# akuhara/RF_INV

Measured on NVIDIA B200. Metric: forward+likelihood evals/sec, higher is better.
Workload: dtype f64

## Files before the change

### rf_inv_b200/csrc/capi.cu

```cuda
#include <cstdarg>
#include <cstdio>
#include <cstdlib>
#include <cstring>
#include <cmath>
#include <vector>
#include <algorithm>
#include "rfinv_handle.h"

static thread_local char g_err[1024] = "";

int rfinv_pdl_mode() {
  static const int mode = getenv("RFINV_PDL") ? atoi(getenv("RFINV_PDL")) : 2;
  return mode;
}

int rfinv_arith_switches() {
  auto on = [](const char* name) { return getenv(name) && atoi(getenv(name)) != 0; };
  static const int bits = (on("RFINV_FULL_BAND") ? 1 : 0) | (on("RFINV_QF_DENSE") ? 2 : 0) | (on("RFINV_QF_NOSPLIT") ? 4 : 0);
  return bits;
}

void rfinv_set_error(const char* fmt, ...) {
  va_list ap;
  va_start(ap, fmt);
// ... 365 lines not shown
  h->h_ipha.assign(cfg->ipha, cfg->ipha + T);
  h->h_obs.assign(cfg->obs, cfg->obs + (size_t)T * S);
  h->h_vp_ref.assign(cfg->vp_ref, cfg->vp_ref + cfg->nref);
  h->h_vs_ref.assign(cfg->vs_ref, cfg->vs_ref + cfg->nref);
  h->h_sig_min.assign(cfg->sig_min, cfg->sig_min + T);
  h->h_sig_max.assign(cfg->sig_max, cfg->sig_max + T);
  if (cfg->r_inv) h->h_r_inv.assign(cfg->r_inv, cfg->r_inv + (size_t)T * S * S);
  else build_r_inv(*cfg, h->h_r_inv);
  h->cfg.rayps = h->h_rayps.data(); h->cfg.a_gus = h->h_a_gus.data(); h->cfg.ipha = h->h_ipha.data();
  h->cfg.obs = h->h_obs.data(); h->cfg.vp_ref = h->h_vp_ref.data(); h->cfg.vs_ref = h->h_vs_ref.data();
  h->cfg.sig_min = h->h_sig_min.data(); h->cfg.sig_max = h->h_sig_max.data(); h->cfg.r_inv = h->h_r_inv.data();

  DevConfig& d = h->dc;
  std::memset(&d, 0, sizeof(d));
  d.ntrc = T; d.nfft = cfg->nfft; d.nh = cfg->nfft / 2 + 1; d.nsmp = S;
  d.nfft_p2 = 64; while (d.nfft_p2 < cfg->nfft) d.nfft_p2 <<= 1;
  d.fft_general = d.nfft_p2 != cfg->nfft;
  d.fft_len = d.fft_general ? 2 * d.nfft_p2 : cfg->nfft;
  d.log2n = 0; while ((1 << d.log2n) < d.fft_len) ++d.log2n;
  d.deconv_mode = cfg->deconv_mode; d.vp_mode = cfg->vp_mode; d.k_min = cfg->k_min; d.k_max = cfg->k_max;
  d.prior_mode = cfg->prior_mode; d.nref = cfg->nref;
  d.ray_common = 1;
  for (int t = 1; t < T; ++t)
    if (cfg->rayps[t] != cfg->rayps[0] || cfg->ipha[t] != cfg->ipha[0]) d.ray_common = 0;
  d.nsmp_pad = ((S + 63) / 64) * 64;
  d.delta = cfg->delta; d.t_start = cfg->t_start; d.sdep = cfg->sdep; d.bdep = cfg->bdep; d.z_ref_min = cfg->z_ref_min; d.dz_ref = cfg->dz_ref;
  d.z_min = cfg->z_min; d.z_max = cfg->z_max; d.h_min = cfg->h_min;
  d.vp_min = cfg->vp_min; d.vp_max = cfg->vp_max; d.vs_min = cfg->vs_min; d.vs_max = cfg->vs_max;
  d.vpvs_min = cfg->vpvs_min; d.vpvs_max = cfg->vpvs_max;
  d.domg = 2.0 * RFINV_PI / (cfg->nfft * cfg->delta);
  for (int t = 0; t < T; ++t) { d.rayp[t] = cfg->rayps[t]; d.ipha[t] = cfg->ipha[t]; }

  std::vector<double> flt;
  build_filter(*cfg, flt);
  band_limits(d, flt);
  std::vector<double2> tw;
  build_twiddles(d.fft_len, tw);
  std::vector<double2> chirp, chirp_b;
  std::vector<double2> twq;
  if (d.fft_general) {
    build_chirp(cfg->nfft, d.fft_len, chirp, chirp_b);
    for (int N = d.fft_len; N > 8; N >>= 3) {
      const int stride = N >> 3, tmul = d.fft_len / N;
      for (int i = 0; i < 7 * stride; ++i) { const int q = i / stride + 1, o = i - (q - 1) * stride; twq.push_back(tw[(size_t)q * o * tmul]); }
    }
  }
  const int Sp = d.nsmp_pad;
  std::vector<double> rpad((size_t)T * Sp * Sp, 0.0);
  for (int t = 0; t < T; ++t)
    for (int i = 0; i < S; ++i)
      for (int j = 0; j < S; ++j)
        rpad[((size_t)t * Sp + i) * Sp + j] =
            0.5 * (h->h_r_inv[((size_t)t * S + i) * S + j] + h->h_r_inv[((size_t)t * S + j) * S + i]);
  std::vector<double> wfac;
  {
    const bool force_dense = (rfinv_arith_switches() & 2) != 0;
    const bool no_split = (rfinv_arith_switches() & 4) != 0;
    const int ntile_dense = Sp / 64;
    std::vector<std::vector<double>> Wt(T);
    std::vector<int> wrows_t(T, 0);
    std::vector<double> a, w, v, a2, w2, v2;
    d.qf_tiles_max = 0;
    int wrows = 64;
    const double rs2 = 0.70710678118654752440;
    for (int t = 0; t < T; ++t) {
      d.qf_rank[t] = 0; d.qf_rank_s[t] = 0; d.qf_split[t] = 0;
      d.qf_tiles[t] = ntile_dense;
      const double* Rm = &rpad[(size_t)t * Sp * Sp];
      auto R = [&](int i, int j) { return Rm[(size_t)i * Sp + j]; };
      int same = -1;
      for (int u = 0; u < t && same < 0; ++u)
        if (std::memcmp(&rpad[(size_t)u * Sp * Sp], Rm, sizeof(double) * (size_t)Sp * Sp) == 0) same = u;
      if (force_dense) {  }
      else if (same >= 0) {
        d.qf_rank[t] = d.qf_rank[same]; d.qf_rank_s[t] = d.qf_rank_s[same]; d.qf_split[t] = d.qf_split[same];
        d.qf_tiles[t] = d.qf_tiles[same]; Wt[t] = Wt[same]; wrows_t[t] = wrows_t[same];
      } else {
        double rmax = 0.0, asym = 0.0;
        for (int i = 0; i < S; ++i)
          for (int j = 0; j < S; ++j) {
            rmax = std::max(rmax, std::fabs(R(i, j)));
            asym = std::max(asym, std::fabs(R(i, j) - R(S - 1 - i, S - 1 - j)));
          }
        const int ha = S / 2, hs = S - ha;
        const bool split = !no_split && rmax > 0.0 && asym <= 1e-10 * rmax && hs <= Sp / 2;
        const double units_dense = 0.5 * ntile_dense * (ntile_dense + 1);
        auto tile_units = [&](int r) { return r / 64 + (r % 64 ? 0.4 : 0.0); };
        if (split) {
          a.assign((size_t)hs * hs, 0.0); a2.assign((size_t)ha * ha, 0.0);
          for (int i = 0; i < ha; ++i)
            for (int j = 0; j < ha; ++j) {
              const int ir = S - 1 - i, jr = S - 1 - j;
              a[(size_t)i * hs + j] = 0.5 * ((R(i, j) + R(ir, jr)) + (R(i, jr) + R(ir, j)));
              a2[(size_t)i * ha + j] = 0.5 * ((R(i, j) + R(ir, jr)) - (R(i, jr) + R(ir, j)));
            }
          if (hs > ha) {
            const int c = ha;
            a[(size_t)c * hs + c] = R(c, c);
            for (int i = 0; i < ha; ++i) a[(size_t)i * hs + c] = a[(size_t)c * hs + i] = rs2 * (R(i, c) + R(S - 1 - i, c));
          }
          sym_eigh(a, hs, w, v);
          if (ha > 0) sym_eigh(a2, ha, w2, v2); else { w2.clear(); v2.clear(); }
          double lmax = 0.0, lmin = 0.0;
          for (double x : w) { lmax = std::max(lmax, x); lmin = std::min(lmin, x); }
          for (double x : w2) { lmax = std::max(lmax, x); lmin = std::min(lmin, x); }
          const double tol = 1e-12 * lmax;
          std::vector<int> os, oa;
// ... 7 lines not shown
            d.qf_rank[t] = rs + ra; d.qf_rank_s[t] = rs; d.qf_split[t] = 1;
            d.qf_tiles[t] = ts + ta;
            wrows_t[t] = 64 * (ts + ta);
            Wt[t].assign((size_t)wrows_t[t] * Sp, 0.0);
            for (int row = 0; row < rs; ++row) {
              const int e = os[row];
              const double sc = std::sqrt(w[e]);
              double* dst = &Wt[t][(size_t)row * Sp];
              for (int i = 0; i < ha; ++i) dst[i] = sc * rs2 * v[(size_t)i * hs + e];
              if (hs > ha) dst[ha] = sc * v[(size_t)ha * hs + e];
            }
            for (int row = 0; row < ra; ++row) {
              const int e = oa[row];
              const double sc = std::sqrt(w2[e]);
              double* dst = &Wt[t][(size_t)(64 * ts + row) * Sp + Sp / 2];
              for (int i = 0; i < ha; ++i) dst[i] = sc * rs2 * v2[(size_t)i * ha + e];
            }
          }
        }
        if (d.qf_rank[t] == 0 && rmax > 0.0) {
          a.resize((size_t)S * S);
          for (int i = 0; i < S; ++i)
            for (int j = 0; j < S; ++j) a[(size_t)i * S + j] = R(i, j);
          sym_eigh(a, S, w, v);
          double lmax = 0.0, lmin = 0.0;
          for (int e = 0; e < S; ++e) { lmax = std::max(lmax, w[e]); lmin = std::min(lmin, w[e]); }
          const double tol = 1e-12 * lmax;
          int r = 0;
          for (int e = 0; e < S; ++e) r += w[e] > tol;
          if (lmax > 0.0 && lmin >= -tol && r > 0 && tile_units(r) * ntile_dense < 0.9 * units_dense) {
            d.qf_rank[t] = r;
            d.qf_tiles[t] = (r + 63) / 64;
            wrows_t[t] = 64 * d.qf_tiles[t];
            Wt[t].assign((size_t)wrows_t[t] * Sp, 0.0);
            std::vector<int> order;
            for (int e = 0; e < S; ++e) if (w[e] > tol) order.push_back(e);
            std::sort(order.begin(), order.end(), [&](int x, int y) { return w[x] > w[y] || (w[x] == w[y] && x < y); });
            for (int row = 0; row < r; ++row) {
              const int e = order[row];
              const double sc = std::sqrt(w[e]);
              for (int i = 0; i < S; ++i) Wt[t][(size_t)row * Sp + i] = sc * v[(size_t)i * S + e];
            }
          }
        }
      }
      d.qf_tiles_max = std::max(d.qf_tiles_max, d.qf_tiles[t]);
      wrows = std::max(wrows, wrows_t[t]);
    }
    d.qf_wrows = wrows;
    wfac.assign((size_t)T * wrows * Sp, 0.0);
    for (int t = 0; t < T; ++t)
      if (!Wt[t].empty()) std::memcpy(&wfac[(size_t)t * wrows * Sp], Wt[t].data(), sizeof(double) * Wt[t].size());
    {
      int tr = 0;
      for (int t = 0; t < T; ++t) if (d.qf_tiles[t] > d.qf_tiles[tr]) tr = t;
      std::vector<std::pair<double, int>> cost;
      for (int jt = 0; jt < d.qf_tiles_max && jt < RFINV_MAX_QF_TILES; ++jt) {
        double cst;
        if (d.qf_rank[tr] == 0) cst = jt + 1;
        else if (d.qf_split[tr]) {
          const int rs = d.qf_rank_s[tr], ts = (rs + 63) / 64;
          cst = std::min(64, jt < ts ? rs - 64 * jt : (d.qf_rank[tr] - rs) - 64 * (jt - ts));
        } else cst = std::min(64, d.qf_rank[tr] - 64 * jt);
        cost.push_back({-cst, jt});
      }
      std::sort(cost.begin(), cost.end());
      for (size_t q = 0; q < cost.size(); ++q) d.qf_order[q] = cost[q].second;
    }
  }
#define RFINV_TRY(x) do { st = (x); if (st != RFINV_OK) { rfinv_destroy(h); return st; } } while (0)
  RFINV_TRY(upload(flt, &h->d_flt));
  RFINV_TRY(upload(tw, &h->d_tw));
  if (d.fft_general) { RFINV_TRY(upload(chirp, &h->d_chirp)); RFINV_TRY(upload(chirp_b, &h->d_chirp_b)); RFINV_TRY(upload(twq, &h->d_twq)); }
  RFINV_TRY(upload(h->h_obs, &h->d_obs));
  RFINV_TRY(upload(h->h_vp_ref, &h->d_vp_ref));
  RFINV_TRY(upload(h->h_vs_ref, &h->d_vs_ref));
  RFINV_TRY(upload(rpad, &h->d_r_inv));
  RFINV_TRY(upload(wfac, &h->d_w_fac));
#undef RFINV_TRY
  d.flt = h->d_flt; d.tw = h->d_tw; d.chirp = h->d_chirp; d.chirp_b = h->d_chirp_b; d.twq = h->d_twq; d.obs = h->d_obs; d.vp_ref = h->d_vp_ref; d.vs_ref = h->d_vs_ref; d.r_inv = h->d_r_inv; d.w_fac = h->d_w_fac;
  cudaError_t e = cudaStreamCreateWithFlags(&h->stream, cudaStreamNonBlocking);
  if (e != cudaSuccess) { rfinv_set_error("cudaStreamCreate: %s", cudaGetErrorString(e)); rfinv_destroy(h); return RFINV_ERR_CUDA; }
  h->own_stream = true;
  *out = h;
  return RFINV_OK;
}

void rfinv_destroy(rfinv_handle* h) {
  if (!h) return;
  cudaSetDevice(h->device);
  if (h->stream) cudaStreamSynchronize(h->stream);
  h->free_pt();
  rfinv_comm_destroy(h);
  h->free_workspace();
  cudaFree(h->d_flt); cudaFree(h->d_tw); cudaFree(h->d_chirp); cudaFree(h->d_chirp_b); cudaFree(h->d_twq); cudaFree(h->d_obs); cudaFree(h->d_vp_ref); cudaFree(h->d_vs_ref); cudaFree(h->d_r_inv); cudaFree(h->d_w_fac);
  if (h->own_stream && h->stream) cudaStreamDestroy(h->stream);
  if (h->stream_copy) {
    cudaStreamSynchronize(h->stream_copy);
    cudaStreamDestroy(h->stream_copy);
    for (cudaEvent_t e : h->ev_copy) if (e) cudaEventDestroy(e);
  }
  for (int i = 0; i < RFINV_ASYNC_SLOTS; ++i) {
    if (h->async_stream[i]) { cudaStreamSynchronize(h->async_stream[i]); cudaStreamDestroy(h->async_stream[i]); }
    if (h->async_ws[i]) { h->async_ws[i]->release(); delete h->async_ws[i]; }
  }
  for (int i = 0; i < 4; ++i)
    if (h->ev[i]) cudaEventDestroy(h->ev[i]);
  delete h;
}

int32_t rfinv_set_stream(rfinv_handle* h, uint64_t cuda_stream) {
  if (!h) { rfinv_set_error("handle is NULL"); return RFINV_ERR_ARG; }
  if (h->own_stream && h->stream) { cudaStreamSynchronize(h->stream); cudaStreamDestroy(h->stream); }
  h->stream = reinterpret_cast<cudaStream_t>(cuda_stream);
  h->own_stream = false;
  return RFINV_OK;
}

int32_t rfinv_synchronize(rfinv_handle* h) {
  if (!h) { rfinv_set_error("handle is NULL"); return RFINV_ERR_ARG; }
  RFINV_CUDA_CHECK(cudaStreamSynchronize(h->stream));
  return RFINV_OK;
}

int32_t rfinv_last_launch_count(rfinv_handle* h) { return h ? h->launches : 0; }

int32_t rfinv_set_timing(rfinv_handle* h, int32_t enable) {
  if (!h) { rfinv_set_error("handle is NULL"); return RFINV_ERR_ARG; }
  RFINV_CUDA_CHECK(cudaSetDevice(h->device));
  if (enable && !h->ev[0])
    for (int i = 0; i < 4; ++i) RFINV_CUDA_CHECK(cudaEventCreate(&h->ev[i]));
  h->timing = enable != 0;
  return RFINV_OK;
}

int32_t rfinv_get_quadform_form(rfinv_handle* h, int32_t* rank, int32_t* rank_s, int32_t* split) {
  if (!h || !rank || !rank_s || !split) { rfinv_set_error("rfinv_get_quadform_form: NULL argument"); return RFINV_ERR_ARG; }
  for (int t = 0; t < h->dc.ntrc; ++t) { rank[t] = h->dc.qf_rank[t]; rank_s[t] = h->dc.qf_rank_s[t]; split[t] = h->dc.qf_split[t]; }
  return RFINV_OK;
}

int32_t rfinv_get_timing(rfinv_handle* h, double* ms) {
  if (!h || !ms) { rfinv_set_error("NULL argument"); return RFINV_ERR_ARG; }
  if (!h->timing) { rfinv_set_error("rfinv_get_timing: call rfinv_set_timing(h, 1) first"); return RFINV_ERR_STATE; }
  RFINV_CUDA_CHECK(cudaEventSynchronize(h->ev[3]));
  for (int i = 0; i < 3; ++i) {
    float f = 0.f;
    RFINV_CUDA_CHECK(cudaEventElapsedTime(&f, h->ev[i], h->ev[i + 1]));
// ... 305 lines not shown
```

### rf_inv_b200/csrc/likelihood.cu

```cuda
#include "rfinv_common.cuh"

namespace {

constexpr int TM = 64;
constexpr int TN = 64;
constexpr int TK = 16;
constexpr int LDS_STRIDE = TK + 4;
constexpr int QF_THREADS = 128;
constexpr int QF_CHUNK = 384;

__device__ __forceinline__ void cp_async16(void* smem_dst, const void* gmem_src) {
  const unsigned d = (unsigned)__cvta_generic_to_shared(smem_dst);
  asm volatile("cp.async.cg.shared.global [%0], [%1], 16;\n" ::"r"(d), "l"(gmem_src));
}
__device__ __forceinline__ void cp_async_commit() { asm volatile("cp.async.commit_group;\n" ::); }
template <int N>
__device__ __forceinline__ void cp_async_wait() { asm volatile("cp.async.wait_group %0;\n" ::"n"(N)); }

__device__ __forceinline__ void dmma884(double& c0, double& c1, double a, double b) {
  asm volatile("mma.sync.aligned.m8n8k4.row.col.f64.f64.f64.f64 {%0,%1}, {%2}, {%3}, {%0,%1};\n"
               : "+d"(c0), "+d"(c1) : "d"(a), "d"(b));
}

__global__ void __launch_bounds__(QF_THREADS, 4) quadform_kernel(const DevConfig cfg, int C, const double* __restrict__ misfit,
                                                              double* __restrict__ phi, double* __restrict__ partial,
                                                              int* __restrict__ arrivals, int* __restrict__ work,
                                                              const int* __restrict__ active, int n_active,
                                                              const int* __restrict__ n_active_dev, const double* __restrict__ sig,
                                                              double* __restrict__ logl) {
  __shared__ __align__(16) double sA[2][TM * LDS_STRIDE];
  __shared__ __align__(16) double sB[2][TN * LDS_STRIDE];
  __shared__ int s_rows[TM];
  __shared__ double s_part[2][TM];
  __shared__ int s_next, s_last;
  const int Sp = cfg.nsmp_pad, T = cfg.ntrc;
  const int tid = threadIdx.x, lane = tid & 31, warp = tid >> 5;
  const int wm = warp >> 1, wn = warp & 1;
  const int n_rb_grid = ((active ? n_active : C) + TM - 1) / TM;
  const int ntile = cfg.qf_tiles_max;
  const int n_items = ntile * T * n_rb_grid;
  const int fr = lane >> 2, fk = lane & 3;
  if (tid == 0) s_next = (int)gridDim.x + atomicAdd(work, 1);
  pdl_wait();
  const int n_rows = active ? (n_active_dev ? *n_active_dev : n_active) : C;
  int item = blockIdx.x;
  while (item < n_items) {
    const int nblk = T * n_rb_grid;
    const int chunk = item / (ntile * QF_CHUNK), local = item - chunk * (ntile * QF_CHUNK);
    const int cb = min(QF_CHUNK, nblk - chunk * QF_CHUNK);
    const int jt = cfg.qf_order[local / cb];
    const int blk = chunk * QF_CHUNK + local % cb;
    const int t = blk / n_rb_grid, rb = blk - t * n_rb_grid;
    const int row0 = rb * TM;
    const int rank = cfg.qf_rank[t];
    const int ntile_t = cfg.qf_tiles[t];
    __syncthreads();
    const int next = s_next;
    int next_raw = 0;
    if (tid == 0) next_raw = atomicAdd(work, 1);
    if (row0 < n_rows && jt < ntile_t) {
      if (tid < TM) {
        int r = row0 + tid;
        r = r < n_rows ? r : n_rows - 1;
        s_rows[tid] = active ? active[r] : r;
      }
      __syncthreads();
      const double* __restrict__ Mt = misfit + (size_t)t * C * Sp;
      const double* __restrict__ Rt = rank > 0 ? cfg.w_fac + (size_t)t * cfg.qf_wrows * Sp : cfg.r_inv + (size_t)t * Sp * Sp;
      int jw = 4, koff = 0, nk = (jt + 1) * (TN / TK);
      if (rank > 0) {
        int cols_tile = rank - jt * TN;
        nk = Sp / TK;
        if (cfg.qf_split[t]) {
          const int rs = cfg.qf_rank_s[t], ts = (rs + TN - 1) / TN;
          cols_tile = jt < ts ? rs - jt * TN : (rank - rs) - (jt - ts) * TN;
          koff = jt < ts ? 0 : Sp >> 1;
          nk = (Sp >> 1) / TK;
        }
        const int nfrag = cols_tile >= TN ? 8 : (cols_tile <= 0 ? 0 : (cols_tile + 7) >> 3);
        jw = (nfrag + 1 - wn) >> 1;
      }
      const double* a_src[4];
      int cp_off[4], cp_row[4];
#pragma unroll
      for (int q = 0; q < 4; ++q) {
        const int id = tid + q * QF_THREADS;
        const int row = id >> 3, seg = id & 7;
        cp_row[q] = row;
        cp_off[q] = row * LDS_STRIDE + seg * 2;
        a_src[q] = Mt + (size_t)s_rows[row] * Sp + seg * 2 + koff;
      }
      double acc[4][4][2];
#pragma unroll
      for (int i = 0; i < 4; ++i)
#pragma unroll
        for (int j = 0; j < 4; ++j) acc[i][j][0] = acc[i][j][1] = 0.0;
      const double* b_base = Rt + (size_t)(jt * TN) * Sp + koff;
#pragma unroll
      for (int q = 0; q < 4; ++q) {
        cp_async16(&sA[0][cp_off[q]], a_src[q]);
        cp_async16(&sB[0][cp_off[q]], b_base + (size_t)cp_row[q] * Sp + (cp_off[q] - cp_row[q] * LDS_STRIDE));
      }
      cp_async_commit();
      for (int ks = 0; ks < nk; ++ks) {
        const int cur = ks & 1;
        cp_async_wait<0>();
        __syncthreads();
        if (ks + 1 < nk) {
          const int k0 = (ks + 1) * TK;
#pragma unroll
          for (int q = 0; q < 4; ++q) {
            cp_async16(&sA[cur ^ 1][cp_off[q]], a_src[q] + k0);
            cp_async16(&sB[cur ^ 1][cp_off[q]], b_base + (size_t)cp_row[q] * Sp + k0 + (cp_off[q] - cp_row[q] * LDS_STRIDE));
          }
          cp_async_commit();
        }
        if (rank == 0 && ks == jt * (TN / TK) && jt > 0) {
#pragma unroll
          for (int i = 0; i < 4; ++i)
#pragma unroll
            for (int j = 0; j < 4; ++j) { acc[i][j][0] *= 2.0; acc[i][j][1] *= 2.0; }
        }
        const double* A = &sA[cur][(wm * 32 + fr) * LDS_STRIDE + fk];
        const double* B = &sB[cur][(wn * 8 + fr) * LDS_STRIDE + fk];
#pragma unroll
        for (int kk = 0; kk < TK; kk += 4) {
          double a[4], b[4];
#pragma unroll
          for (int i = 0; i < 4; ++i) a[i] = A[i * 8 * LDS_STRIDE + kk];
#pragma unroll
          for (int j = 0; j < 4; ++j) b[j] = B[j * 16 * LDS_STRIDE + kk];
          if (jw == 4) {
#pragma unroll
            for (int i = 0; i < 4; ++i)
#pragma unroll
              for (int j = 0; j < 4; ++j) dmma884(acc[i][j][0], acc[i][j][1], a[i], b[j]);
          } else {
#pragma unroll
            for (int j = 0; j < 4; ++j)
              if (j < jw) {
#pragma unroll
                for (int i = 0; i < 4; ++i) dmma884(acc[i][j][0], acc[i][j][1], a[i], b[j]);
              }
          }
        }
      }
#pragma unroll
      for (int i = 0; i < 4; ++i) {
        const double* mrow = Mt + (size_t)s_rows[wm * 32 + 8 * i + fr] * Sp + jt * TN + wn * 8 + 2 * fk;
        double v = 0.0;
        if (rank > 0) {
#pragma unroll
          for (int j = 0; j < 4; ++j) { v = fma(acc[i][j][0], acc[i][j][0], v); v = fma(acc[i][j][1], acc[i][j][1], v); }
        } else {
#pragma unroll
          for (int j = 0; j < 4; ++j) {
            const double2 m = *reinterpret_cast<const double2*>(mrow + 16 * j);
            v = fma(acc[i][j][0], m.x, v);
            v = fma(acc[i][j][1], m.y, v);
          }
        }
        v += __shfl_xor_sync(0xffffffffu, v, 1);
        v += __shfl_xor_sync(0xffffffffu, v, 2);
        if (fk == 0) s_part[wn][wm * 32 + 8 * i + fr] = v;
      }
      __syncthreads();
      double* part_t = partial + (size_t)t * C;
      const size_t jstride = (size_t)T * C;
      if (tid < TM && row0 + tid < n_rows) part_t[(size_t)jt * jstride + s_rows[tid]] = s_part[0][tid] + s_part[1][tid];
      __threadfence();
      __syncthreads();
      if (tid == 0) s_last = (atomicAdd(&arrivals[t * n_rb_grid + rb], 1) == ntile_t - 1);
      __syncthreads();
      if (s_last) {
        __threadfence();
        if (tid < TM && row0 + tid < n_rows) {
          const int c = s_rows[tid];
          double v = 0.0;
          for (int j = 0; j < ntile_t; ++j) v += __ldcg(part_t + (size_t)j * jstride + c);
          phi[(size_t)t * C + c] = v;
        }
        if (tid == 0) arrivals[t * n_rb_grid + rb] = 0;
        if (logl) {
          __threadfence();
          __syncthreads();
          if (tid == 0) s_last = (atomicAdd(&arrivals[T * n_rb_grid + rb], 1) == T - 1);
          __syncthreads();
          if (s_last) {
            __threadfence();
            if (tid < TM && row0 + tid < n_rows) {
              const int c = s_rows[tid];
              double ll = 0.0;
              for (int tt = 0; tt < T; ++tt) {
                const double sg = sig[(size_t)tt * C + c];
                const double ph = __ldcg(phi + (size_t)tt * C + c);
                ll = __dsub_rn(__dsub_rn(ll, __ddiv_rn(__dmul_rn(0.5, ph), __dmul_rn(sg, sg))), __dmul_rn((double)cfg.nsmp, log(sg)));
              }
              logl[c] = ll;
            }
            if (tid == 0) arrivals[T * n_rb_grid + rb] = 0;
          }
        }
      }
    } else {
      __syncthreads();
    }
    if (tid == 0) s_next = (int)gridDim.x + next_raw;
    item = next;
  }
  if (tid == 0) {
    __threadfence();
    if (atomicAdd(work + 1, 1) == (int)gridDim.x - 1) { work[0] = 0; work[1] = 0; }
  }
}

__global__ void loglik_kernel(const DevConfig cfg, int C, const double* __restrict__ phi, const double* __restrict__ sig,
                              double* __restrict__ logl) {
  const int c = blockIdx.x * blockDim.x + threadIdx.x;
  if (c >= C) return;
  double ll = 0.0;
  for (int t = 0; t < cfg.ntrc; ++t) {
    const double s = sig[(size_t)t * C + c];
    const double ph = phi[(size_t)t * C + c];
    ll = __dsub_rn(__dsub_rn(ll, __ddiv_rn(__dmul_rn(0.5, ph), __dmul_rn(s, s))), __dmul_rn((double)cfg.nsmp, log(s)));
  }
  logl[c] = ll;
}

}

size_t rfinv_quadform_partial_doubles(const DevConfig& cfg, int C) { return (size_t)(cfg.nsmp_pad / TN + 1) * cfg.ntrc * C; }
size_t rfinv_quadform_counter_ints(const DevConfig& cfg, int C) { return (size_t)((C + TM - 1) / TM) * (cfg.ntrc + 1) + 4; }

int rfinv_launch_quadform(const DevConfig& cfg, int C, const double* misfit, double* phi, double* partial, int* counters,
                          const int* active, int n_active, const int* n_active_dev, cudaStream_t stream, const double* sig,
                          double* logl) {
  const int n_rows = active ? n_active : C;
  if (n_rows == 0) return RFINV_OK;
  const size_t ntile = cfg.qf_tiles_max;
  int* work = counters;
  int* arrivals = counters + 4;
  static int resident_of_device[64] = {0};
  int dev = 0;
  RFINV_CUDA_CHECK(cudaGetDevice(&dev));
  long long resident = (dev >= 0 && dev < 64) ? resident_of_device[dev] : 0;
  if (resident == 0) {
    int per_sm = 0, n_sm = 0;
    RFINV_CUDA_CHECK(cudaDeviceGetAttribute(&n_sm, cudaDevAttrMultiProcessorCount, dev));
    RFINV_CUDA_CHECK(cudaOccupancyMaxActiveBlocksPerMultiprocessor(&per_sm, quadform_kernel, QF_THREADS, 0));
    resident = (long long)n_sm * (per_sm < 1 ? 1 : per_sm);
    if (dev >= 0 && dev < 64) resident_of_device[dev] = (int)resident;
  }
  const long long items = (long long)ntile * cfg.ntrc * ((n_rows + TM - 1) / TM);
  RFINV_CUDA_CHECK(rfinv_launch_pdl(2, quadform_kernel, dim3((unsigned)(items < resident ? items : resident)), dim3(QF_THREADS), 0, stream, cfg, C,
                                    misfit, phi, partial, arrivals, work, active, n_active, n_active_dev, sig, logl));
  return RFINV_OK;
}

int rfinv_launch_loglik(const DevConfig& cfg, int C, const double* phi, const double* sig, double* logl,
                        cudaStream_t stream) {
  if (C == 0) return RFINV_OK;
  loglik_kernel<<<(C + 255) / 256, 256, 0, stream>>>(cfg, C, phi, sig, logl);
  RFINV_CUDA_CHECK(cudaGetLastError());
  return RFINV_OK;
}
```

### rf_inv_b200/csrc/rfinv_common.cuh

```cuda
#pragma once
#include <cuda_runtime.h>
#include <stdint.h>
#include <math.h>
#include <map>
#include <mutex>
#include <utility>
#include "../../include/rfinv_b200.h"

#define RFINV_MAX_TRC 16
#define RFINV_MAX_K 64
#define RFINV_MAX_LAY (RFINV_MAX_K + 2)
#define RFINV_MAX_QF_TILES 64

#define RFINV_PI 3.1415926535897931

struct DevConfig {
  int ntrc, nfft, nh, nsmp;
  int log2n;
  int fft_general, nfft_p2, fft_len;
  int deconv_mode, vp_mode, k_min, k_max, prior_mode, nref, ray_common;
  int nsmp_pad;
  double bdep;
  double delta, t_start, sdep, z_ref_min, dz_ref, z_min, z_max, h_min;
  double vp_min, vp_max, vs_min, vs_max, vpvs_min, vpvs_max;
  double domg;
  double rayp[RFINV_MAX_TRC];
  int ipha[RFINV_MAX_TRC];
  int jbins[RFINV_MAX_TRC];
  int jb_max;
  const double* flt;
  const double2* tw;
  const double2* twq;
  const double2* chirp;
  const double2* chirp_b;
  const double* obs;
  const double* vp_ref;
  const double* vs_ref;
  const double* r_inv;
  const double* w_fac;
  int qf_rank[RFINV_MAX_TRC];
  int qf_split[RFINV_MAX_TRC];
  int qf_rank_s[RFINV_MAX_TRC];
  int qf_tiles[RFINV_MAX_TRC];
  int qf_tiles_max, qf_wrows;
  int qf_order[RFINV_MAX_QF_TILES];
};

struct ModelBatch {
  int C;
  const int* k;
  const double* z;
  const double* dvp;
  const double* dvs;
  const double* sig;
  const int* active;
  int n_active;
  const int* n_active_dev;
  int chain_major = 0;
};

__host__ __device__ __forceinline__ int f_nint(double x) {
  return x >= 0.0 ? (int)floor(x + 0.5) : -(int)floor(-x + 0.5);
}

__device__ __forceinline__ double vp_to_rho(double a1) {
  double a2 = __dmul_rn(a1, a1), a3 = __dmul_rn(a2, a1), a4 = __dmul_rn(a3, a1), a5 = __dmul_rn(a4, a1);
  double p = __dmul_rn((double)1.6612f, a1);
  p = __dsub_rn(p, __dmul_rn((double)0.4721f, a2));
  p = __dadd_rn(p, __dmul_rn((double)0.0671f, a3));
  p = __dsub_rn(p, __dmul_rn((double)0.0043f, a4));
  p = __dadd_rn(p, __dmul_rn((double)0.000106f, a5));
  return p;
}

__device__ __forceinline__ bool layer_velocity(const DevConfig& cfg, double zc, double d_vs, double d_vp, double& alpha,
                                               double& beta) {
  int iz = f_nint(__ddiv_rn(__dsub_rn(zc, cfg.z_ref_min), cfg.dz_ref)) + 1;
  iz = iz < 1 ? 1 : (iz > cfg.nref ? cfg.nref : iz);
  beta = __dadd_rn(cfg.vs_ref[iz - 1], d_vs);
  alpha = cfg.vp_mode == 1 ? __dadd_rn(cfg.vp_ref[iz - 1], d_vp) : cfg.vp_ref[iz - 1];
  double ratio = __ddiv_rn(alpha, beta);
  return !(alpha < cfg.vp_min || alpha > cfg.vp_max || beta < cfg.vs_min || beta > cfg.vs_max ||
           ratio < cfg.vpvs_min || ratio > cfg.vpvs_max);
}

#define RFINV_CUDA_CHECK(expr)                                                        \
  do {                                                                                \
    cudaError_t e__ = (expr);                                                         \
    if (e__ != cudaSuccess) {                                                         \
      rfinv_set_error("%s:%d: %s -> %s", __FILE__, __LINE__, #expr, cudaGetErrorString(e__)); \
      return RFINV_ERR_CUDA;                                                          \
    }                                                                                 \
  } while (0)

void rfinv_set_error(const char* fmt, ...);

inline cudaError_t rfinv_raise_smem_limit(const void* kernel, size_t bytes) {
  static std::mutex mu;
// ... 55 lines not shown
```

### rf_inv_b200/csrc/rfinv_handle.h

```cpp
#pragma once
#include <vector>
#include "rfinv_common.cuh"

struct PtState;

struct EvalWorkspace {
  int cap = 0;
  int* d_k = nullptr;
  double *d_z = nullptr, *d_dvp = nullptr, *d_dvs = nullptr, *d_sig = nullptr, *d_stage = nullptr;
  double *d_misfit = nullptr, *d_phi = nullptr, *d_logl = nullptr, *d_rft_full = nullptr, *d_scratch = nullptr;
  uint8_t* d_valid = nullptr;
  double* d_qpart = nullptr;
  int* d_qcnt = nullptr;
  size_t cap_rft_full = 0;
  int grow(const DevConfig& dc, const rfinv_config& cfg, int device, int C);
  void release();
};

constexpr int RFINV_ASYNC_SLOTS = 2;
constexpr int RFINV_UPLOAD_PIECES = 4;

struct rfinv_handle : EvalWorkspace {
  int device = 0;
  cudaStream_t stream = nullptr;
  bool own_stream = false;
  rfinv_config cfg;
  std::vector<double> h_rayps, h_a_gus, h_obs, h_vp_ref, h_vs_ref, h_sig_min, h_sig_max, h_r_inv;
  std::vector<int32_t> h_ipha;
  DevConfig dc;
  double* d_flt = nullptr;
  double2* d_tw = nullptr;
  double2 *d_chirp = nullptr, *d_chirp_b = nullptr, *d_twq = nullptr;
  double* d_obs = nullptr;
  double* d_vp_ref = nullptr;
  double* d_vs_ref = nullptr;
  double* d_r_inv = nullptr;
  double* d_w_fac = nullptr;
  cudaStream_t stream_copy = nullptr;
  cudaEvent_t ev_copy[RFINV_UPLOAD_PIECES + 2] = {};
  EvalWorkspace* async_ws[RFINV_ASYNC_SLOTS] = {};
  cudaStream_t async_stream[RFINV_ASYNC_SLOTS] = {};
  bool async_pending[RFINV_ASYNC_SLOTS] = {};
  int launches = 0;
  bool timing = false;
  cudaEvent_t ev[4] = {nullptr, nullptr, nullptr, nullptr};
  PtState* pt = nullptr;
  void* comm = nullptr;
  int comm_world = 1, comm_rank = 0;

  int ensure_capacity(int C) { if (C > cap) invalidate_pt_graphs(); return grow(dc, cfg, device, C); }
  void invalidate_pt_graphs();
  void free_workspace() { release(); }
  void free_pt();
  int eval_device(int C, const int* k, const double* z, const double* dvp, const double* dvs, const double* sig,
                  double* logl, double* rft_smp, double* rft_full, uint8_t* is_valid, const int* active, int n_active,
                  const ModelBatch* layout = nullptr, EvalWorkspace* w = nullptr, cudaStream_t s = nullptr,
                  bool prep_done = false,
                  cudaEvent_t before_quadform = nullptr);
};

int rfinv_comm_allgather(rfinv_handle* h, const double* send, double* recv, size_t count, cudaStream_t s);
extern "C" int32_t rfinv_comm_destroy(rfinv_handle* h);
int rfinv_comm_peer_setup(rfinv_handle* h);
void rfinv_comm_peer_release(rfinv_handle* h);
int rfinv_pt_fix_assigned_bins(rfinv_handle* h);
int rfinv_pt_reserve_lhist(rfinv_handle* h, int upto);
int rfinv_arith_switches();
```

Baseline: 12.93 million.

## Emulate FP64 low-rank quadratic form with int8 tcgen05 slice GEMMs

Adds a new quadform kernel for low-rank factored traces. The misfit rows and precomputed weight factors are split into 7 int8 byte slices with per-row and per-column exponent scaling, multiplied on Blackwell tcgen05 int8 MMA into TMEM, and recombined into doubles. Rows holding non-finite values fall back to an exact FP64 loop. The old DMMA kernel now handles only dense traces, and the two kernels split the fused logl reduction. This aims to replace slow FP64 tensor-core throughput with much faster int8 throughput. It costs preprocessing, extra launch complexity and possible accuracy differences from truncating the fixed-point slices.

```diff
diff --git a/rf_inv_b200/csrc/capi.cu b/rf_inv_b200/csrc/capi.cu
--- a/rf_inv_b200/csrc/capi.cu
+++ b/rf_inv_b200/csrc/capi.cu
@@ -441,7 +441,8 @@
       for (int j = 0; j < S; ++j)
         rpad[((size_t)t * Sp + i) * Sp + j] =
             0.5 * (h->h_r_inv[((size_t)t * S + i) * S + j] + h->h_r_inv[((size_t)t * S + j) * S + i]);
-  std::vector<double> wfac;
+  std::vector<double> wfac, wcolf;
+  std::vector<uint8_t> wi8;
   {
     const bool force_dense = (rfinv_arith_switches() & 2) != 0;
     const bool no_split = (rfinv_arith_switches() & 4) != 0;
@@ -555,6 +556,31 @@
     for (int t = 0; t < T; ++t)
       if (!Wt[t].empty()) std::memcpy(&wfac[(size_t)t * wrows * Sp], Wt[t].data(), sizeof(double) * Wt[t].size());
     {
+      const int ntw = wrows / 64, nks = Sp / 32;
+      wi8.assign((size_t)T * ntw * nks * 7 * 2048, 0);
+      wcolf.assign((size_t)T * wrows, 0.0);
+      for (int t = 0; t < T; ++t) {
+        if (d.qf_rank[t] == 0) continue;
+        for (int e = 0; e < wrows; ++e) {
+          const double* col = &wfac[((size_t)t * wrows + e) * Sp];
+          double mx = 0.0;
+          for (int k = 0; k < Sp; ++k) mx = std::max(mx, std::fabs(col[k]));
+          if (mx == 0.0) continue;
+          int ec = 0;
+          std::frexp(mx, &ec);
+          wcolf[(size_t)t * wrows + e] = std::ldexp(1.0, ec - 30);
+          const int jt = e / 64, c = e % 64;
+          for (int k = 0; k < Sp; ++k) {
+            const long long X = std::llrint(std::ldexp(col[k], 55 - ec));
+            const int ks = k / 32, kb = k % 32;
+            uint8_t* blk = &wi8[(((size_t)t * ntw + jt) * nks + ks) * 7 * 2048];
+            const size_t off = (size_t)(c / 8) * 256 + (kb / 16) * 128 + (c % 8) * 16 + kb % 16;
+            for (int p = 0; p < 7; ++p) blk[(size_t)p * 2048 + off] = (uint8_t)((unsigned long long)X >> (8 * (6 - p)));
+          }
+        }
+      }
+    }
+    {
       int tr = 0;
       for (int t = 0; t < T; ++t) if (d.qf_tiles[t] > d.qf_tiles[tr]) tr = t;
       std::vector<std::pair<double, int>> cost;
@@ -580,8 +606,11 @@
   RFINV_TRY(upload(h->h_vs_ref, &h->d_vs_ref));
   RFINV_TRY(upload(rpad, &h->d_r_inv));
   RFINV_TRY(upload(wfac, &h->d_w_fac));
+  RFINV_TRY(upload(wi8, &h->d_w_i8));
+  RFINV_TRY(upload(wcolf, &h->d_w_colf));
 #undef RFINV_TRY
   d.flt = h->d_flt; d.tw = h->d_tw; d.chirp = h->d_chirp; d.chirp_b = h->d_chirp_b; d.twq = h->d_twq; d.obs = h->d_obs; d.vp_ref = h->d_vp_ref; d.vs_ref = h->d_vs_ref; d.r_inv = h->d_r_inv; d.w_fac = h->d_w_fac;
+  d.w_i8 = h->d_w_i8; d.w_colf = h->d_w_colf;
   cudaError_t e = cudaStreamCreateWithFlags(&h->stream, cudaStreamNonBlocking);
   if (e != cudaSuccess) { rfinv_set_error("cudaStreamCreate: %s", cudaGetErrorString(e)); rfinv_destroy(h); return RFINV_ERR_CUDA; }
   h->own_stream = true;
@@ -597,6 +626,7 @@
   rfinv_comm_destroy(h);
   h->free_workspace();
   cudaFree(h->d_flt); cudaFree(h->d_tw); cudaFree(h->d_chirp); cudaFree(h->d_chirp_b); cudaFree(h->d_twq); cudaFree(h->d_obs); cudaFree(h->d_vp_ref); cudaFree(h->d_vs_ref); cudaFree(h->d_r_inv); cudaFree(h->d_w_fac);
+  cudaFree(h->d_w_i8); cudaFree(h->d_w_colf);
   if (h->own_stream && h->stream) cudaStreamDestroy(h->stream);
   if (h->stream_copy) {
     cudaStreamSynchronize(h->stream_copy);
diff --git a/rf_inv_b200/csrc/likelihood.cu b/rf_inv_b200/csrc/likelihood.cu
--- a/rf_inv_b200/csrc/likelihood.cu
+++ b/rf_inv_b200/csrc/likelihood.cu
@@ -58,7 +58,7 @@
     const int next = s_next;
     int next_raw = 0;
     if (tid == 0) next_raw = atomicAdd(work, 1);
-    if (row0 < n_rows && jt < ntile_t) {
+    if (row0 < n_rows && jt < ntile_t && rank == 0) {
       if (tid < TM) {
         int r = row0 + tid;
         r = r < n_rows ? r : n_rows - 1;
@@ -66,20 +66,8 @@
       }
       __syncthreads();
       const double* __restrict__ Mt = misfit + (size_t)t * C * Sp;
-      const double* __restrict__ Rt = rank > 0 ? cfg.w_fac + (size_t)t * cfg.qf_wrows * Sp : cfg.r_inv + (size_t)t * Sp * Sp;
-      int jw = 4, koff = 0, nk = (jt + 1) * (TN / TK);
-      if (rank > 0) {
-        int cols_tile = rank - jt * TN;
-        nk = Sp / TK;
-        if (cfg.qf_split[t]) {
-          const int rs = cfg.qf_rank_s[t], ts = (rs + TN - 1) / TN;
-          cols_tile = jt < ts ? rs - jt * TN : (rank - rs) - (jt - ts) * TN;
-          koff = jt < ts ? 0 : Sp >> 1;
-          nk = (Sp >> 1) / TK;
-        }
-        const int nfrag = cols_tile >= TN ? 8 : (cols_tile <= 0 ? 0 : (cols_tile + 7) >> 3);
-        jw = (nfrag + 1 - wn) >> 1;
-      }
+      const double* __restrict__ Rt = cfg.r_inv + (size_t)t * Sp * Sp;
+      const int nk = (jt + 1) * (TN / TK);
       const double* a_src[4];
       int cp_off[4], cp_row[4];
 #pragma unroll
@@ -88,14 +76,14 @@
         const int row = id >> 3, seg = id & 7;
         cp_row[q] = row;
         cp_off[q] = row * LDS_STRIDE + seg * 2;
-        a_src[q] = Mt + (size_t)s_rows[row] * Sp + seg * 2 + koff;
+        a_src[q] = Mt + (size_t)s_rows[row] * Sp + seg * 2;
       }
       double acc[4][4][2];
 #pragma unroll
       for (int i = 0; i < 4; ++i)
 #pragma unroll
         for (int j = 0; j < 4; ++j) acc[i][j][0] = acc[i][j][1] = 0.0;
-      const double* b_base = Rt + (size_t)(jt * TN) * Sp + koff;
+      const double* b_base = Rt + (size_t)(jt * TN) * Sp;
 #pragma unroll
       for (int q = 0; q < 4; ++q) {
         cp_async16(&sA[0][cp_off[q]], a_src[q]);
@@ -115,7 +103,7 @@
           }
           cp_async_commit();
         }
-        if (rank == 0 && ks == jt * (TN / TK) && jt > 0) {
+        if (ks == jt * (TN / TK) && jt > 0) {
 #pragma unroll
           for (int i = 0; i < 4; ++i)
 #pragma unroll
@@ -130,35 +118,21 @@
           for (int i = 0; i < 4; ++i) a[i] = A[i * 8 * LDS_STRIDE + kk];
 #pragma unroll
           for (int j = 0; j < 4; ++j) b[j] = B[j * 16 * LDS_STRIDE + kk];
-          if (jw == 4) {
-#pragma unroll
-            for (int i = 0; i < 4; ++i)
-#pragma unroll
-              for (int j = 0; j < 4; ++j) dmma884(acc[i][j][0], acc[i][j][1], a[i], b[j]);
-          } else {
-#pragma unroll
-            for (int j = 0; j < 4; ++j)
-              if (j < jw) {
-#pragma unroll
-                for (int i = 0; i < 4; ++i) dmma884(acc[i][j][0], acc[i][j][1], a[i], b[j]);
-              }
-          }
+#pragma unroll
+          for (int i = 0; i < 4; ++i)
+#pragma unroll
+            for (int j = 0; j < 4; ++j) dmma884(acc[i][j][0], acc[i][j][1], a[i], b[j]);
         }
       }
 #pragma unroll
       for (int i = 0; i < 4; ++i) {
         const double* mrow = Mt + (size_t)s_rows[wm * 32 + 8 * i + fr] * Sp + jt * TN + wn * 8 + 2 * fk;
         double v = 0.0;
-        if (rank > 0) {
-#pragma unroll
-          for (int j = 0; j < 4; ++j) { v = fma(acc[i][j][0], acc[i][j][0], v); v = fma(acc[i][j][1], acc[i][j][1], v); }
-        } else {
-#pragma unroll
-          for (int j = 0; j < 4; ++j) {
-            const double2 m = *reinterpret_cast<const double2*>(mrow + 16 * j);
-            v = fma(acc[i][j][0], m.x, v);
-            v = fma(acc[i][j][1], m.y, v);
-          }
+#pragma unroll
+        for (int j = 0; j < 4; ++j) {
+          const double2 m = *reinterpret_cast<const double2*>(mrow + 16 * j);
+          v = fma(acc[i][j][0], m.x, v);
+          v = fma(acc[i][j][1], m.y, v);
         }
         v += __shfl_xor_sync(0xffffffffu, v, 1);
         v += __shfl_xor_sync(0xffffffffu, v, 2);
@@ -227,33 +201,373 @@
   logl[c] = ll;
 }
 
+
+constexpr int Q8_TM = 128;
+constexpr int Q8_TN = 64;
+constexpr int Q8_TK = 32;
+constexpr int Q8_SL = 7;
+constexpr int Q8_THREADS = 256;
+constexpr int Q8_STAGES = 3;
+constexpr int Q8_CHUNK = 192;
+constexpr int Q8_A_BYTES = Q8_TM * Q8_TK;
+constexpr int Q8_B_BYTES = Q8_TN * Q8_TK;
+constexpr int Q8_STAGE_BYTES = Q8_SL * (Q8_A_BYTES + Q8_B_BYTES);
+constexpr int Q8_SMEM = Q8_STAGES * Q8_STAGE_BYTES;
+constexpr uint32_t Q8_TMEM_COLS = 512;
+#ifndef RFINV_Q8_LBO
+#define RFINV_Q8_LBO 128
+#endif
+#ifndef RFINV_Q8_SBO
+#define RFINV_Q8_SBO 256
+#endif
+constexpr uint32_t Q8_IDESC = (2u << 4) | ((uint32_t)(Q8_TN >> 3) << 17) | ((uint32_t)(Q8_TM >> 4) << 24);
+
+__device__ __forceinline__ uint32_t smem_u32(const void* p) { return (uint32_t)__cvta_generic_to_shared(p); }
+__device__ __forceinline__ uint64_t umma_desc(uint32_t saddr) {
+  return (uint64_t)((saddr & 0x3FFFFu) >> 4) | ((uint64_t)(RFINV_Q8_LBO >> 4) << 16) | ((uint64_t)(RFINV_Q8_SBO >> 4) << 32) |
+         (1ull << 46);
+}
+__device__ __forceinline__ void mbar_wait(uint64_t* bar, uint32_t parity) {
+  const uint32_t a = smem_u32(bar);
+  uint32_t done = 0;
+  do {
+    asm volatile("{\n.reg .pred p;\nmbarrier.try_wait.parity.shared::cta.b64 p, [%1], %2;\nselp.u32 %0, 1, 0, p;\n}\n"
+                 : "=r"(done) : "r"(a), "r"(parity) : "memory");
+  } while (!done);
+}
+__device__ __forceinline__ void tc_fence_before() { asm volatile("tcgen05.fence::before_thread_sync;" ::: "memory"); }
+__device__ __forceinline__ void tc_fence_after() { asm volatile("tcgen05.fence::after_thread_sync;" ::: "memory"); }
+__device__ __forceinline__ void mma_i8(uint32_t d_tmem, uint64_t a_desc, uint64_t b_desc, uint32_t idesc, uint32_t acc) {
+  asm volatile("{\n.reg .pred p;\nsetp.ne.b32 p, %4, 0;\ntcgen05.mma.cta_group::1.kind::i8 [%0], %1, %2, %3, p;\n}\n"
+               :: "r"(d_tmem), "l"(a_desc), "l"(b_desc), "r"(idesc), "r"(acc) : "memory");
+}
+__device__ __forceinline__ void tmem_ld8(uint32_t taddr, int (&v)[8]) {
+  asm volatile("tcgen05.ld.sync.aligned.32x32b.x8.b32 {%0, %1, %2, %3, %4, %5, %6, %7}, [%8];"
+               : "=r"(v[0]), "=r"(v[1]), "=r"(v[2]), "=r"(v[3]), "=r"(v[4]), "=r"(v[5]), "=r"(v[6]), "=r"(v[7]) : "r"(taddr));
+}
+__device__ __forceinline__ double i2d_exact(long long x) {
+  return __longlong_as_double(0x4338000000000000LL + x) - 6755399441055744.0;
+}
+
+__global__ void __launch_bounds__(Q8_THREADS, 1) quadform_i8_kernel(const DevConfig cfg, int C, const double* __restrict__ misfit,
+                                                                 double* __restrict__ phi, double* __restrict__ partial,
+                                                                 int* __restrict__ arrivals, int* __restrict__ work,
+                                                                 const int* __restrict__ active, int n_active,
+                                                                 const int* __restrict__ n_active_dev, const double* __restrict__ sig,
+                                                                 double* __restrict__ logl, int n_fac) {
+  extern __shared__ __align__(128) uint8_t q8_smem[];
+  __shared__ __align__(8) uint64_t s_bar[Q8_STAGES];
+  __shared__ uint32_t s_tmem;
+  __shared__ int s_rows[Q8_TM], s_exp[Q8_TM], s_bad[Q8_TM];
+  __shared__ uint32_t s_hmax[Q8_TM];
+  __shared__ double s_part[2][Q8_TM];
+  __shared__ int s_next, s_last;
+  const int Sp = cfg.nsmp_pad, T = cfg.ntrc;
+  const int tid = threadIdx.x, lane = tid & 31, warp = tid >> 5;
+  const int n_rb_grid = ((active ? n_active : C) + Q8_TM - 1) / Q8_TM;
+  const int ntile = cfg.qf_tiles_max;
+  const int n_items = ntile * T * n_rb_grid;
+  const int ntw = cfg.qf_wrows / Q8_TN, nks = Sp / Q8_TK;
+  if (warp == 0) {
+    asm volatile("tcgen05.alloc.cta_group::1.sync.aligned.shared::cta.b32 [%0], %1;" :: "r"(smem_u32(&s_tmem)), "r"(Q8_TMEM_COLS) : "memory");
+    asm volatile("tcgen05.relinquish_alloc_permit.cta_group::1.sync.aligned;" ::: "memory");
+  }
+  if (tid == 0) {
+    for (int s = 0; s < Q8_STAGES; ++s) asm volatile("mbarrier.init.shared::cta.b64 [%0], 1;" :: "r"(smem_u32(&s_bar[s])) : "memory");
+    asm volatile("fence.mbarrier_init.release.cluster;" ::: "memory");
+    s_next = (int)gridDim.x + atomicAdd(work, 1);
+  }
+  tc_fence_before();
+  __syncthreads();
+  tc_fence_after();
+  const uint32_t tmem = s_tmem;
+  pdl_wait();
+  const int n_rows = active ? (n_active_dev ? *n_active_dev : n_active) : C;
+  uint32_t step = 0;
+  int item = blockIdx.x;
+  while (item < n_items) {
+    const int nblk = T * n_rb_grid;
+    const int chunk = item / (ntile * Q8_CHUNK), local = item - chunk * (ntile * Q8_CHUNK);
+    const int cb = min(Q8_CHUNK, nblk - chunk * Q8_CHUNK);
+    const int jt = cfg.qf_order[local / cb];
+    const int blk = chunk * Q8_CHUNK + local % cb;
+    const int t = blk / n_rb_grid, rb = blk - t * n_rb_grid;
+    const int row0 = rb * Q8_TM;
+    const int rank = cfg.qf_rank[t];
+    const int ntile_t = cfg.qf_tiles[t];
+    __syncthreads();
+    const int next = s_next;
+    int next_raw = 0;
+    if (tid == 0) next_raw = atomicAdd(work, 1);
+    if (row0 < n_rows && jt < ntile_t && rank > 0) {
+      if (tid < Q8_TM) {
+        int r = row0 + tid;
+        r = r < n_rows ? r : n_rows - 1;
+        s_rows[tid] = active ? active[r] : r;
+      }
+      int cols_tile = rank - jt * Q8_TN, koff = 0, klen = Sp;
+      if (cfg.qf_split[t]) {
+        const int rs = cfg.qf_rank_s[t], ts = (rs + Q8_TN - 1) / Q8_TN;
+        cols_tile = jt < ts ? rs - jt * Q8_TN : (rank - rs) - (jt - ts) * Q8_TN;
+        koff = jt < ts ? 0 : Sp >> 1;
+        klen = Sp >> 1;
+      }
+      const int nk = klen / Q8_TK;
+      const double* __restrict__ Mt = misfit + (size_t)t * C * Sp;
+      __syncthreads();
+      if (tid < Q8_TM) s_hmax[tid] = 0u;
+      __syncthreads();
+      {
+        const int dpr = klen >> 1, total = Q8_TM * dpr;
+        for (int base = 0; base < total; base += 16 * Q8_THREADS) {
+          uint32_t hm[16];
+          int rw[16];
+#pragma unroll
+          for (int u = 0; u < 16; ++u) {
+            const int idx = base + u * Q8_THREADS + tid;
+            const int row = idx < total ? idx / dpr : 0;
+            rw[u] = row;
+            hm[u] = 0u;
+            if (idx < total) {
+              const double2 v = __ldg(reinterpret_cast<const double2*>(Mt + (size_t)s_rows[row] * Sp + koff + 2 * (idx - row * dpr)));
+              hm[u] = max((uint32_t)__double2hiint(v.x) & 0x7FFFFFFFu, (uint32_t)__double2hiint(v.y) & 0x7FFFFFFFu);
+            }
+          }
+#pragma unroll
+          for (int u = 0; u < 16; ++u) {
+            uint32_t h = hm[u];
+#pragma unroll
+            for (int o = 1; o < 16; o <<= 1) h = max(h, __shfl_xor_sync(0xffffffffu, h, o));
+            if ((lane & 15) == 0 && h) atomicMax(&s_hmax[rw[u]], h);
+          }
+        }
+      }
+      __syncthreads();
+      if (tid < Q8_TM) {
+        const uint32_t hmax = s_hmax[tid];
+        const int E = (int)(hmax >> 20);
+        s_exp[tid] = E == 0 ? -1022 : E - 1022;
+        s_bad[tid] = hmax >= 0x7FF00000u;
+      }
+      __syncthreads();
+      const double* a_src[4];
+      double sc1[4], sc2[4];
+      int a_off[4];
+#pragma unroll
+      for (int i = 0; i < 4; ++i) {
+        const int row = (tid >> 3) + 32 * i, g = tid & 7;
+        a_src[i] = Mt + (size_t)s_rows[row] * Sp + koff + 4 * g;
+        const int sx = 55 - s_exp[row];
+        const int s1 = min(sx, 1000);
+        sc1[i] = __longlong_as_double((long long)(1023 + s1) << 52);
+        sc2[i] = __longlong_as_double((long long)(1023 + sx - s1) << 52);
+        a_off[i] = (row >> 3) * RFINV_Q8_SBO + (g >> 2) * RFINV_Q8_LBO + (row & 7) * 16 + (g & 3) * 4;
+      }
+      const uint8_t* b_src = cfg.w_i8 + (((size_t)t * ntw + jt) * nks + (koff / Q8_TK)) * (size_t)(Q8_SL * Q8_B_BYTES);
+      double2 cur[4][2], nxt[4][2];
+#pragma unroll
+      for (int i = 0; i < 4; ++i) {
+        cur[i][0] = __ldg(reinterpret_cast<const double2*>(a_src[i]));
+        cur[i][1] = __ldg(reinterpret_cast<const double2*>(a_src[i] + 2));
+      }
+      for (int ks = 0; ks < nk; ++ks, ++step) {
+        const uint32_t stage = step % Q8_STAGES;
+        uint8_t* sA = q8_smem + stage * Q8_STAGE_BYTES;
+        uint8_t* sB = sA + Q8_SL * Q8_A_BYTES;
+        if (step >= Q8_STAGES) mbar_wait(&s_bar[stage], ((step / Q8_STAGES) - 1) & 1);
+        {
+          const uint8_t* src = b_src + (size_t)ks * (Q8_SL * Q8_B_BYTES);
+          for (int c = tid; c < Q8_SL * Q8_B_BYTES / 16; c += Q8_THREADS) cp_async16(sB + 16 * c, src + 16 * c);
+          cp_async_commit();
+        }
+        if (ks + 1 < nk) {
+#pragma unroll
+          for (int i = 0; i < 4; ++i) {
+            nxt[i][0] = __ldg(reinterpret_cast<const double2*>(a_src[i] + (ks + 1) * Q8_TK));
+            nxt[i][1] = __ldg(reinterpret_cast<const double2*>(a_src[i] + (ks + 1) * Q8_TK + 2));
+          }
+        }
+#pragma unroll
+        for (int i = 0; i < 4; ++i) {
+          const double x[4] = {cur[i][0].x, cur[i][0].y, cur[i][1].x, cur[i][1].y};
+          uint32_t lo[4], hi[4];
+#pragma unroll
+          for (int j = 0; j < 4; ++j) {
+            const long long X = __double2ll_rn(__dmul_rn(__dmul_rn(x[j], sc1[i]), sc2[i]));
+            lo[j] = (uint32_t)X;
+            hi[j] = (uint32_t)((unsigned long long)X >> 32);
+          }
+          uint8_t* dst = sA + a_off[i];
+          uint32_t u01 = __byte_perm(lo[0], lo[1], 0x5140), u23 = __byte_perm(lo[2], lo[3], 0x5140);
+          *reinterpret_cast<uint32_t*>(dst + 6 * Q8_A_BYTES) = __byte_perm(u01, u23, 0x5410);
+          *reinterpret_cast<uint32_t*>(dst + 5 * Q8_A_BYTES) = __byte_perm(u01, u23, 0x7632);
+          u01 = __byte_perm(lo[0], lo[1], 0x7362); u23 = __byte_perm(lo[2], lo[3], 0x7362);
+          *reinterpret_cast<uint32_t*>(dst + 4 * Q8_A_BYTES) = __byte_perm(u01, u23, 0x5410);
+          *reinterpret_cast<uint32_t*>(dst + 3 * Q8_A_BYTES) = __byte_perm(u01, u23, 0x7632);
+          u01 = __byte_perm(hi[0], hi[1], 0x5140); u23 = __byte_perm(hi[2], hi[3], 0x5140);
+          *reinterpret_cast<uint32_t*>(dst + 2 * Q8_A_BYTES) = __byte_perm(u01, u23, 0x5410);
+          *reinterpret_cast<uint32_t*>(dst + 1 * Q8_A_BYTES) = __byte_perm(u01, u23, 0x7632);
+          u01 = __byte_perm(hi[0], hi[1], 0x7362); u23 = __byte_perm(hi[2], hi[3], 0x7362);
+          *reinterpret_cast<uint32_t*>(dst) = __byte_perm(u01, u23, 0x5410);
+        }
+        cp_async_wait<0>();
+        asm volatile("fence.proxy.async.shared::cta;" ::: "memory");
+        __syncthreads();
+        if (tid == 0) {
+          tc_fence_after();
+          const uint32_t a0 = smem_u32(sA), b0 = smem_u32(sB);
+#pragma unroll
+          for (int L = 0; L < Q8_SL; ++L)
+#pragma unroll
+            for (int p = 0; p <= L; ++p) {
+              const int q = L - p;
+              mma_i8(tmem + L * Q8_TN, umma_desc(a0 + p * Q8_A_BYTES), umma_desc(b0 + q * Q8_B_BYTES),
+                     Q8_IDESC | (p == 0 ? 1u << 7 : 0u) | (q == 0 ? 1u << 10 : 0u), (ks > 0 || p > 0) ? 1u : 0u);
+            }
+          asm volatile("tcgen05.commit.cta_group::1.mbarrier::arrive::one.shared::cluster.b64 [%0];"
+                       :: "r"(smem_u32(&s_bar[stage])) : "memory");
+        }
+#pragma unroll
+        for (int i = 0; i < 4; ++i) { cur[i][0] = nxt[i][0]; cur[i][1] = nxt[i][1]; }
+      }
+      mbar_wait(&s_bar[(step - 1) % Q8_STAGES], ((step - 1) / Q8_STAGES) & 1);
+      tc_fence_after();
+      const int qd = warp & 3, h = warp >> 2, r = 32 * qd + lane;
+      const double* colf = cfg.w_colf + (size_t)t * cfg.qf_wrows + jt * Q8_TN + 32 * h;
+      double v = 0.0;
+#pragma unroll
+      for (int c8 = 0; c8 < 4; ++c8) {
+        int acc[Q8_SL][8];
+#pragma unroll
+        for (int L = 0; L < Q8_SL; ++L) tmem_ld8(tmem + ((uint32_t)(32 * qd) << 16) + L * Q8_TN + 32 * h + 8 * c8, acc[L]);
+        asm volatile("tcgen05.wait::ld.sync.aligned;" ::: "memory");
+#pragma unroll
+        for (int j = 0; j < 8; ++j) {
+          const long long g0 = ((long long)acc[0][j] << 16) + ((long long)acc[1][j] << 8) + acc[2][j];
+          const long long g1 = ((long long)acc[3][j] << 16) + ((long long)acc[4][j] << 8) + acc[5][j];
+          const double y = __dmul_rn(fma(i2d_exact(acc[6][j]), 0x1p-32, fma(i2d_exact(g1), 0x1p-24, i2d_exact(g0))), colf[8 * c8 + j]);
+          v = fma(y, y, v);
+        }
+      }
+      tc_fence_before();
+      v = scalbn(v, 2 * s_exp[r]);
+      if (s_bad[r]) {
+        const int ncol = min(Q8_TN, (cols_tile + 7) & ~7);
+        const double* m = Mt + (size_t)s_rows[r] * Sp + koff;
+        v = 0.0;
+        for (int c = 32 * h; c < min(32 * h + 32, ncol); ++c) {
+          const double* w = cfg.w_fac + ((size_t)t * cfg.qf_wrows + jt * Q8_TN + c) * Sp + koff;
+          double y = 0.0;
+          for (int k = 0; k < klen; ++k) y = fma(m[k], w[k], y);
+          v = fma(y, y, v);
+        }
+      }
+      s_part[h][r] = v;
+      __syncthreads();
+      double* part_t = partial + (size_t)t * C;
+      const size_t jstride = (size_t)T * C;
+      if (tid < Q8_TM && row0 + tid < n_rows) part_t[(size_t)jt * jstride + s_rows[tid]] = s_part[0][tid] + s_part[1][tid];
+      __threadfence();
+      __syncthreads();
+      if (tid == 0) s_last = (atomicAdd(&arrivals[t * n_rb_grid + rb], 1) == ntile_t - 1);
+      __syncthreads();
+      if (s_last) {
+        __threadfence();
+        if (tid < Q8_TM && row0 + tid < n_rows) {
+          const int c = s_rows[tid];
+          double v2 = 0.0;
+          for (int j = 0; j < ntile_t; ++j) v2 += __ldcg(part_t + (size_t)j * jstride + c);
+          phi[(size_t)t * C + c] = v2;
+        }
+        if (tid == 0) arrivals[t * n_rb_grid + rb] = 0;
+        if (logl) {
+          __threadfence();
+          __syncthreads();
+          if (tid == 0) s_last = (atomicAdd(&arrivals[T * n_rb_grid + rb], 1) == n_fac - 1);
+          __syncthreads();
+          if (s_last) {
+            __threadfence();
+            if (tid < Q8_TM && row0 + tid < n_rows) {
+              const int c = s_rows[tid];
+              double ll = 0.0;
+              for (int tt = 0; tt < T; ++tt) {
+                const double sg = sig[(size_t)tt * C + c];
+                const double ph = __ldcg(phi + (size_t)tt * C + c);
+                ll = __dsub_rn(__dsub_rn(ll, __ddiv_rn(__dmul_rn(0.5, ph), __dmul_rn(sg, sg))), __dmul_rn((double)cfg.nsmp, log(sg)));
+              }
+              logl[c] = ll;
+            }
+            if (tid == 0) arrivals[T * n_rb_grid + rb] = 0;
+          }
+        }
+      }
+    } else {
+      __syncthreads();
+    }
+    if (tid == 0) s_next = (int)gridDim.x + next_raw;
+    item = next;
+  }
+  if (tid == 0) {
+    __threadfence();
+    if (atomicAdd(work + 1, 1) == (int)gridDim.x - 1) { work[0] = 0; work[1] = 0; }
+  }
+  tc_fence_before();
+  __syncthreads();
+  if (warp == 0) {
+    tc_fence_after();
+    asm volatile("tcgen05.dealloc.cta_group::1.sync.aligned.b32 %0, %1;" :: "r"(tmem), "r"(Q8_TMEM_COLS) : "memory");
+  }
+}
+
 }
 
 size_t rfinv_quadform_partial_doubles(const DevConfig& cfg, int C) { return (size_t)(cfg.nsmp_pad / TN + 1) * cfg.ntrc * C; }
 size_t rfinv_quadform_counter_ints(const DevConfig& cfg, int C) { return (size_t)((C + TM - 1) / TM) * (cfg.ntrc + 1) + 4; }
+
+template <typename K>
+static int resident_ctas(K kernel, int threads, size_t smem, int (&cache)[64], long long& resident) {
+  int dev = 0;
+  RFINV_CUDA_CHECK(cudaGetDevice(&dev));
+  resident = (dev >= 0 && dev < 64) ? cache[dev] : 0;
+  if (resident == 0) {
+    int per_sm = 0, n_sm = 0;
+    RFINV_CUDA_CHECK(cudaDeviceGetAttribute(&n_sm, cudaDevAttrMultiProcessorCount, dev));
+    RFINV_CUDA_CHECK(cudaOccupancyMaxActiveBlocksPerMultiprocessor(&per_sm, kernel, threads, smem));
+    resident = (long long)n_sm * (per_sm < 1 ? 1 : per_sm);
+    if (dev >= 0 && dev < 64) cache[dev] = (int)resident;
+  }
+  return RFINV_OK;
+}
 
 int rfinv_launch_quadform(const DevConfig& cfg, int C, const double* misfit, double* phi, double* partial, int* counters,
                           const int* active, int n_active, const int* n_active_dev, cudaStream_t stream, const double* sig,
                           double* logl) {
   const int n_rows = active ? n_active : C;
   if (n_rows == 0) return RFINV_OK;
-  const size_t ntile = cfg.qf_tiles_max;
-  int* work = counters;
+  int n_fac = 0;
+  for (int t = 0; t < cfg.ntrc; ++t) n_fac += cfg.qf_rank[t] > 0;
   int* arrivals = counters + 4;
-  static int resident_of_device[64] = {0};
-  int dev = 0;
-  RFINV_CUDA_CHECK(cudaGetDevice(&dev));
-  long long resident = (dev >= 0 && dev < 64) ? resident_of_device[dev] : 0;
-  if (resident == 0) {
-    int per_sm = 0, n_sm = 0;
-    RFINV_CUDA_CHECK(cudaDeviceGetAttribute(&n_sm, cudaDevAttrMultiProcessorCount, dev));
-    RFINV_CUDA_CHECK(cudaOccupancyMaxActiveBlocksPerMultiprocessor(&per_sm, quadform_kernel, QF_THREADS, 0));
-    resident = (long long)n_sm * (per_sm < 1 ? 1 : per_sm);
-    if (dev >= 0 && dev < 64) resident_of_device[dev] = (int)resident;
-  }
-  const long long items = (long long)ntile * cfg.ntrc * ((n_rows + TM - 1) / TM);
-  RFINV_CUDA_CHECK(rfinv_launch_pdl(2, quadform_kernel, dim3((unsigned)(items < resident ? items : resident)), dim3(QF_THREADS), 0, stream, cfg, C,
-                                    misfit, phi, partial, arrivals, work, active, n_active, n_active_dev, sig, logl));
+  if (n_fac < cfg.ntrc) {
+    static int cache[64] = {0};
+    long long resident = 0;
+    const int st = resident_ctas(quadform_kernel, QF_THREADS, 0, cache, resident);
+    if (st != RFINV_OK) return st;
+    const long long items = (long long)cfg.qf_tiles_max * cfg.ntrc * ((n_rows + TM - 1) / TM);
+    RFINV_CUDA_CHECK(rfinv_launch_pdl(2, quadform_kernel, dim3((unsigned)(items < resident ? items : resident)), dim3(QF_THREADS), 0, stream, cfg, C,
+                                      misfit, phi, partial, arrivals, counters, active, n_active, n_active_dev, sig,
+                                      n_fac ? nullptr : logl));
+  }
+  if (n_fac > 0) {
+    static int cache[64] = {0};
+    long long resident = 0;
+    RFINV_CUDA_CHECK(rfinv_raise_smem_limit((const void*)quadform_i8_kernel, Q8_SMEM));
+    const int st = resident_ctas(quadform_i8_kernel, Q8_THREADS, Q8_SMEM, cache, resident);
+    if (st != RFINV_OK) return st;
+    const long long items = (long long)cfg.qf_tiles_max * cfg.ntrc * ((n_rows + Q8_TM - 1) / Q8_TM);
+    RFINV_CUDA_CHECK(rfinv_launch_pdl(2, quadform_i8_kernel, dim3((unsigned)(items < resident ? items : resident)), dim3(Q8_THREADS), Q8_SMEM, stream,
+                                      cfg, C, misfit, phi, partial, arrivals, counters + 2, active, n_active, n_active_dev, sig,
+                                      logl, n_fac));
+  }
   return RFINV_OK;
 }
 
diff --git a/rf_inv_b200/csrc/rfinv_common.cuh b/rf_inv_b200/csrc/rfinv_common.cuh
--- a/rf_inv_b200/csrc/rfinv_common.cuh
+++ b/rf_inv_b200/csrc/rfinv_common.cuh
@@ -44,6 +44,8 @@
   int qf_tiles[RFINV_MAX_TRC];
   int qf_tiles_max, qf_wrows;
   int qf_order[RFINV_MAX_QF_TILES];
+  const uint8_t* w_i8;
+  const double* w_colf;
 };
 
 struct ModelBatch {
diff --git a/rf_inv_b200/csrc/rfinv_handle.h b/rf_inv_b200/csrc/rfinv_handle.h
--- a/rf_inv_b200/csrc/rfinv_handle.h
+++ b/rf_inv_b200/csrc/rfinv_handle.h
@@ -36,6 +36,8 @@
   double* d_vs_ref = nullptr;
   double* d_r_inv = nullptr;
   double* d_w_fac = nullptr;
+  uint8_t* d_w_i8 = nullptr;
+  double* d_w_colf = nullptr;
   cudaStream_t stream_copy = nullptr;
   cudaEvent_t ev_copy[RFINV_UPLOAD_PIECES + 2] = {};
   EvalWorkspace* async_ws[RFINV_ASYNC_SLOTS] = {};
```

After: 9.699 million, median of 6. 0.75x the previous value.
